# Contingencyy/CPUGPUPathtracing

Hardware: AMD Instinct MI355X
Metric: Mrays/sec @ 1920x1080, 256 spp (dragon glTF stand-in) (higher is better)
Workload: dtype f32

## Files before the change

cpugpupathtracing_amd/_native.py:

```python
from __future__ import annotations

import ctypes as C
import os

from ._paths import LIB_PATH

ABI_VERSION = 2
CGPT_OK, CGPT_ERR_INVALID, CGPT_ERR_HIP, CGPT_ERR_NO_SCENE, CGPT_ERR_UNSUPPORTED, CGPT_ERR_NO_DEVICE = range(6)
OBJECT_MESH, OBJECT_SPHERE, OBJECT_PLANE, OBJECT_TRIANGLE = 0, 1, 2, 3
MODE_COMPARISON, MODE_BRUTE_FORCE, MODE_ADVANCED = 0, 1, 2
DEBUG_NONE, DEBUG_RAY_DEPTH, DEBUG_BVH_DEPTH = 0, 1, 2
KERNEL_AUTO, KERNEL_MEGAKERNEL, KERNEL_WAVEFRONT, KERNEL_PERSISTENT = 0, 1, 2, 3
RENDER_COUNTERS = 1
CTX_FORCE_COLLECTIVE, CTX_GATHER_PEER_COPY = 1, 2
BUILD_NAIVE, BUILD_SAH_INTERVALS, BUILD_SAH_PRIMITIVES = 0, 1, 2
BUILD_SAH_BINNED = 3
DENOISE_DEMODULATE_ALBEDO = 1
TRACE_COUNTERS, TRACE_REVERSED = 1, 2
TEMPORAL_KEEP_VIEW_DEPENDENT = 1

f3 = C.c_float * 3


class Vertex(C.Structure):
# ... 145 lines not shown
    "cgpt_denoise": (C.c_int, [_vp, C.POINTER(Camera), C.POINTER(DenoiseParams), _fp, C.c_size_t, _up, C.c_size_t]),
    "cgpt_denoise_temporal": (C.c_int, [_vp, C.POINTER(Camera), C.POINTER(DenoiseParams), C.POINTER(TemporalParams), _fp, C.c_size_t, _up,
                                        C.c_size_t]),
    "cgpt_temporal_reset": (C.c_int, [_vp]),
    "cgpt_read_temporal_history": (C.c_int, [_vp, _fp, C.c_size_t]),
    "cgpt_measure_issue_rate": (C.c_int, [_vp, C.c_uint32, C.c_uint32, C.c_uint32, C.POINTER(C.c_double), C.POINTER(C.c_double)]),
    "cgpth_last_error": (C.c_char_p, []),
    "cgpth_mesh_load_gltf": (_vp, [C.c_char_p]),
    "cgpth_mesh_from_arrays": (_vp, [C.POINTER(Vertex), C.c_uint32, _up, C.c_uint32]),
    "cgpth_mesh_dragon_standin": (_vp, [C.c_uint32]),
    "cgpth_mesh_bumpy_icosphere": (_vp, [C.c_uint32, _fp, _fp, C.c_float]),
    "cgpth_mesh_save_gltf": (C.c_int, [_vp, C.c_char_p]),
    "cgpth_mesh_num_vertices": (C.c_uint32, [_vp]),
    "cgpth_mesh_num_indices": (C.c_uint32, [_vp]),
    "cgpth_mesh_vertices": (C.POINTER(Vertex), [_vp]),
    "cgpth_mesh_indices": (_up, [_vp]),
    "cgpth_mesh_free": (None, [_vp]),
    "cgpth_scene_new": (_vp, []),
    "cgpth_scene_free": (None, [_vp]),
    "cgpth_scene_reference_layout": (_vp, [_vp, C.c_uint32, C.c_float, C.c_int]),
    "cgpth_scene_add_material": (C.c_int, [_vp, C.POINTER(Material)]),
    "cgpth_scene_set_material": (C.c_int, [_vp, C.c_uint32, C.POINTER(Material)]),
    "cgpth_scene_set_roughness": (C.c_int, [_vp, C.c_uint32, C.c_float]),
    "cgpth_scene_get_roughness": (C.c_int, [_vp, _fp, C.c_uint32]),
    "cgpth_scene_set_transmission_roughness": (C.c_int, [_vp, C.c_uint32, C.c_float]),
    "cgpth_scene_get_transmission_roughness": (C.c_int, [_vp, _fp, C.c_uint32]),
    "cgpth_scene_add_mesh": (C.c_int, [_vp, _vp, C.c_uint32, C.c_int]),
    "cgpth_scene_add_mesh_device_built": (C.c_int, [_vp, _vp, C.c_uint32, _vp]),
    "cgpth_scene_add_mesh_device_built_ex": (C.c_int, [_vp, _vp, C.c_uint32, _vp, C.c_int]),
    "cgpth_scene_rebuild_bvh_device": (C.c_int, [_vp, C.c_uint32, C.c_int, _vp]),
    "cgpth_scene_add_sphere": (C.c_int, [_vp, _fp, C.c_float, C.c_uint32]),
    "cgpth_scene_add_plane": (C.c_int, [_vp, _fp, _fp, C.c_uint32]),
    "cgpth_scene_add_triangle": (C.c_int, [_vp, C.POINTER(Triangle), C.c_uint32]),
    "cgpth_scene_add_light": (C.c_int, [_vp, C.c_uint32]),
    "cgpth_scene_set_smooth_normals": (C.c_int, [_vp, C.c_uint32, C.c_uint32]),
    "cgpth_scene_get_smooth_normals": (C.c_int, [_vp, _up, C.c_uint32]),
    "cgpth_scene_set_transform": (C.c_int, [_vp, C.c_uint32, C.POINTER(C.c_float)]),
    "cgpth_scene_get_transforms": (C.c_int, [_vp, C.POINTER(C.c_float), C.c_uint32]),
    "cgpth_scene_set_camera": (C.c_int, [_vp, _fp, _fp, C.c_float, C.c_float]),
    "cgpth_scene_set_settings": (C.c_int, [_vp, C.POINTER(Settings)]),
    "cgpth_scene_rebuild_bvh": (C.c_int, [_vp, C.c_uint32, C.c_int]),
    "cgpth_scene_refit_mesh": (C.c_int, [_vp, C.c_uint32, C.POINTER(Triangle), C.c_uint32]),
    "cgpth_scene_update_primitive": (C.c_int, [_vp, C.c_uint32, C.POINTER(Object)]),
    "cgpth_scene_bvh_info": (C.c_int, [_vp, C.c_uint32, C.POINTER(BvhInfo)]),
    "cgpth_scene_bvh_export": (C.c_int, [_vp, C.c_uint32, C.POINTER(BvhNode), _up]),
    "cgpth_scene_flatten": (C.c_int, [_vp, C.POINTER(SceneDesc)]),
    "cgpth_scene_get_camera": (C.c_int, [_vp, C.POINTER(Camera)]),
    "cgpth_scene_get_settings": (C.c_int, [_vp, C.POINTER(Settings)]),
    "cgpth_write_ppm": (C.c_int, [C.c_char_p, _up, C.c_uint32, C.c_uint32]),
    "cgpth_write_pfm": (C.c_int, [C.c_char_p, _fp, C.c_uint32, C.c_uint32, C.c_uint32]),
    "cgpth_write_accumulator": (C.c_int, [C.c_char_p, _fp, C.c_uint32, C.c_uint32, C.c_uint32]),
    "cgpth_read_accumulator": (C.c_int, [C.c_char_p, _fp, _up, C.c_uint32, C.c_uint32]),
    "cgpth_fast_div": (C.c_uint32, [C.c_uint32, C.c_uint32]),
    "cgpth_scene_layout": (C.c_int, [C.POINTER(SceneDesc), C.POINTER(SceneLayoutView)]),
    "cgpth_scene_layout_transformed": (C.c_int, [C.POINTER(SceneDesc), C.POINTER(C.c_float), C.c_uint32, C.POINTER(SceneLayoutView)]),
    "cgpth_scene_permute_objects": (C.c_int, [_vp, _up, C.c_uint32]),
    "cgpth_top_level": (C.c_int, [C.POINTER(SceneDesc), C.POINTER(TopLevelView)]),
    "cgpth_top_level_transforms": (C.c_int, [C.POINTER(C.c_float), C.c_uint32, C.POINTER(TopLevelView)]),
    "cgpth_top_level_refit": (C.c_int, [C.c_uint32, C.POINTER(Triangle), C.c_uint32, C.POINTER(TopLevelView)]),
    "cgpth_top_level_primitive": (C.c_int, [C.c_uint32, C.POINTER(Object), C.POINTER(TopLevelView)]),
}

DEBUG_PROTOTYPES = {
    "cgpt_debug_live_device_bytes": (C.c_uint64, []),
}

_lib = None


class NativeLibraryError(RuntimeError):
    pass


def lib() -> C.CDLL:
    global _lib
    if _lib is not None:
        return _lib
    if not os.path.exists(LIB_PATH):
        raise NativeLibraryError(
            f"{LIB_PATH} is missing: run `python -m cpugpupathtracing_amd.build` (hipcc, gfx950). "
            "There is no CPU or Python fallback for the render path.")
    L = C.CDLL(LIB_PATH)
    for name, (restype, argtypes) in {**PROTOTYPES, **DEBUG_PROTOTYPES}.items():
        try:
            fn = getattr(L, name)
        except AttributeError as e:
            raise NativeLibraryError(f"{LIB_PATH} does not export {name}; rebuild it") from e
        fn.restype = restype
        fn.argtypes = argtypes
    if L.cgpt_abi_version() != ABI_VERSION:
        raise NativeLibraryError(f"ABI version mismatch: library reports {L.cgpt_abi_version()}, binding expects {ABI_VERSION}")
    _lib = L
    return L
```

cpugpupathtracing_amd/csrc/device/accumulate.hpp:

```cpp
#pragma once
#include <hip/hip_runtime.h>

#include "device_scene.h"
#include "rt_device.hpp"
#include "shade_device.hpp"
#include "trace_steps.hpp"

namespace cgpt {
namespace dev {

static constexpr uint32_t kAccChunk = 8;

__device__ __forceinline__ void accumulate_batch(const DevRenderArgs& args, const float4* __restrict__ st_en, const PathGrid& g,
                                                 uint32_t batch_first, uint32_t batch_n)
{
    __shared__ float4 stage[4][64 * (kAccChunk + 1u)];
    const DevSettings& st = args.settings;
    const uint32_t lane = threadIdx.x & 63u;
    float4* const my_stage = stage[threadIdx.x >> 6];
    double energy_sum = 0.0;
    for (uint32_t p = blockIdx.x * 256u + threadIdx.x; p < g.n_pixels; p += gridDim.x * 256u) {
        uint32_t px = 0, py = 0, local_row = 0;
        const bool is_pixel = pixel_of_index(args, g, p, px, py, local_row);
        const size_t local_index = (size_t)local_row * args.width + px;
        const bool brute = st.render_mode == 1u || (st.render_mode == 0u && px < args.width / 2u);
        float4 acc = is_pixel ? args.accumulator[local_index] : float4{ 0.0f, 0.0f, 0.0f, 0.0f };
        V3 last = mk(0.0f);
        auto add_sample = [&](float4 e4) {
            PathState ps;
            ps.energy = mk(e4.x, e4.y, e4.z);
            ps.depth = __float_as_uint(e4.w) & 0xFFu;
            const V3 e = brute ? ps.energy : final_energy(st, ps);
            energy_sum += (double)(e.x + e.y + e.z) * 0.001;
            if (st.debug_mode == 0u) { acc.x += e.x; acc.y += e.y; acc.z += e.z; acc.w += 1.0f; }
            else last = e;
        };
        if (g.order == kPixelMajor) {
            const uint32_t p_base = p - lane;
            for (uint32_t s0 = 0; s0 < batch_n; s0 += kAccChunk) {
                const uint32_t cnt = min(kAccChunk, batch_n - s0);
#pragma unroll
                for (uint32_t k = 0; k < kAccChunk; ++k) {
                    const uint32_t e = k * 64u + lane, pix = e / kAccChunk, smp = e % kAccChunk;
                    if (smp < cnt) my_stage[pix * (kAccChunk + 1u) + smp] = st_en[(size_t)(p_base + pix) * g.n_samples + s0 + smp];
                }
                __builtin_amdgcn_wave_barrier();
                if (is_pixel)
                    for (uint32_t j = 0; j < cnt; ++j) add_sample(my_stage[lane * (kAccChunk + 1u) + j]);
                __builtin_amdgcn_wave_barrier();
            }
        } else if (is_pixel) {
            for (uint32_t s = 0; s < batch_n; ++s) add_sample(ld_stream(&st_en[path_id(g, s, p)]));
        }
        if (is_pixel) {
            if (st.debug_mode == 0u) {
                args.accumulator[local_index] = acc;
                const float n = (float)(batch_first + batch_n);
                args.pixels[local_index] = vec4_to_uint(acc.x / n, acc.y / n, acc.z / n);
            } else {
                args.pixels[local_index] = vec4_to_uint(last.x, last.y, last.z);
            }
        }
    }
    block_add_f64(&args.counters->total_energy, energy_sum);
}

}
}
```

cpugpupathtracing_amd/csrc/device/wavefront_kernels.hip:

```cpp
#include <hip/hip_runtime.h>

#include <algorithm>
#include <cstdint>
#include <cstddef>
#include <cstdlib>
#include <cstring>
#include <new>
#include <type_traits>
#include <vector>

#include "cpugpupt_abi.h"
#include "ctx_internal.h"
#include "device_scene.h"
#include "fast_div.h"
#include "rt_device.hpp"
#include "shade_device.hpp"
#include "trace_steps.hpp"
#include "accumulate.hpp"
#include "launch_common.h"

namespace cgpt {

using namespace dev;

hipStream_t CtxStream(cgpt_ctx* ctx);
void** CtxWavefrontSlot(cgpt_ctx* ctx);
hipEvent_t CtxStartEvent(cgpt_ctx* ctx);

extern __shared__ uint32_t lds_dyn[];

static constexpr uint32_t kMaxBands = 128;

struct WfDev {
    float4* A; float4* B; float4* C;
    float4* st_tp; float4* st_en;
    float4* px_hit;
    float4* brute;
    uint8_t* hit_flag;
    uint32_t* list_ext; uint32_t* list_sh;
    uint32_t* seg_ext; uint32_t* seg_sh;
    uint32_t* seg_count;
    uint32_t* seg_prefix;
    uint32_t n_bands;
    uint32_t band_magic;
    uint32_t* plan;
    uint32_t* stack_overflow;
    uint32_t cap;
    uint32_t n_paths;
    PathGrid g;
    uint32_t n_segs, seg_cap;
    uint32_t shade_chunk;
    uint32_t retire_misses;
    uint32_t rot_trace[2], rot_shade;
    unsigned long long* spec_tab;
    uint32_t spec_keys;
    uint32_t spec_epoch;
    uint32_t probe;
};

static constexpr uint32_t kChainShift = 10u, kChainMax = 0xFFFFu, kFollowerBit = 0x80000000u, kNoLeader = 0xFFFFFFFFu;
static constexpr uint32_t kSameRayBit = 0x40000000u;

__device__ __forceinline__ uint32_t elect_chain_leader(const WfDev& wf, uint32_t chain, uint32_t pid)
{
    const bool want = chain != 0u;
    uint32_t pixel = 0;
    if (want) { uint32_t sample_unused; path_split(wf.g, pid, sample_unused, pixel); }
    uint32_t src = lane_id();
    for (unsigned long long pend = __builtin_amdgcn_ballot_w64(want); pend != 0ull;) {
// ... 155 lines not shown
                do {
                    if (r.code < kStartObject) inner_step<COUNT, STEP>(ctx, r, cnt);
                } while ((uint32_t)__popcll(__builtin_amdgcn_ballot_w64(r.code < kStartObject)) >= tune.inner_repeat);
            } else if (n_leaf >= w_obj) {
                do {
                    if ((int32_t)r.code < 0) leaf_step<COUNT, !FIRST, STEP>(ctx, r, cnt);
                } while ((uint32_t)__popcll(__builtin_amdgcn_ballot_w64((int32_t)r.code < 0)) >= tune.leaf_repeat);
            } else {
                do {
                    if (r.code == kStartObject && object_step<COUNT, !FIRST, XFORM, TREE>(ctx, r, cnt)) finish_ray();
                } while ((uint32_t)__popcll(__builtin_amdgcn_ballot_w64(r.code == kStartObject)) >= tune.obj_repeat);
            }
        }
    }

    const uint32_t per_ray = first_round ? wf.g.n_samples : 1u;
    if (first_round) wave_add_u64(&counters->traced_rays, cnt.rays, per_ray);
    else if (lane_id() == 0u && wave_rays) atomicAdd(&counters->traced_rays, (unsigned long long)wave_rays);
    if (!COUNT && !first_round && lane_id() == 0u && wave_followers) atomicAdd(&counters->chain_followers, (unsigned long long)wave_followers);
    if (!COUNT && !first_round && lane_id() == 0u && wave_unwalked) atomicAdd(&counters->retrace_unwalked, (unsigned long long)wave_unwalked);
    if (COUNT) {
        wave_add_u64(&counters->inner_steps, cnt.inner, per_ray);
        wave_add_u64(&counters->tri_tests, cnt.tris, per_ray);
        wave_add_u64(&counters->bvh_depth_sum, cnt.depth, per_ray);
    }
}

struct ShadeKernArgs { DevRenderArgs args; WfDev wf; uint32_t batch_first; };
static_assert(alignof(DevRenderArgs) == 8 && alignof(WfDev) == 8 && sizeof(DevRenderArgs) % 8 == 0, "ShadeKernArgs mirrors the argument segment: every parameter at its natural alignment");
__device__ __forceinline__ const ShadeKernArgs& shade_kernargs()
{
    const CGPT_UNIFORM ShadeKernArgs* p = (const CGPT_UNIFORM ShadeKernArgs*)__builtin_amdgcn_kernarg_segment_ptr();
    asm volatile("" : "+s"(p));
    return *(const ShadeKernArgs*)p;
}

template <bool COUNT, bool FIRST, bool BRUTE = false, int LOBES = 0, bool RIS = false>
__global__ void __launch_bounds__(256, 1) wf_shade(const DevRenderArgs, const WfDev, uint32_t)
{
    constexpr bool first_round = FIRST;
    constexpr bool kChains = !COUNT && !BRUTE;
    uint32_t n_ext;
    { const WfDev& wf = shade_kernargs().wf; n_ext = first_round ? wf.n_paths : wf.plan[0]; }
    const uint32_t n_blocks = (n_ext + 63u) / 64u;
    const uint32_t n_waves = gridDim.x * 4u;
    const uint32_t wave = blockIdx.x * 4u + __builtin_amdgcn_readfirstlane(threadIdx.x >> 6);
    uint32_t count_ext = 0, count_sh = 0;
    uint32_t cur_band = 0, band_start_ext = 0, band_start_sh = 0;
    Counters cnt = { 0, 0, 0, 0, 0, 0 };
    uint32_t wave_probed = 0;
    uint32_t wave_absorbed = 0;

    BlockWalk walk = first_block(wave);
    uint32_t block = wave * shade_kernargs().wf.shade_chunk;
    auto more = [&]() { return block < n_blocks; };
    auto advance = [&]() {
        const WfDev& wf = shade_kernargs().wf;
        const uint32_t chunk = wf.shade_chunk;
        if (++block >= min((block_of(walk) + 1u) * chunk, n_blocks)) {
            next_block(walk, n_waves, wf.rot_shade);
            block = block_of(walk) * chunk;
        }
    };
    __shared__ uint32_t s_queue[4][128];
    uint32_t* const queue = s_queue[threadIdx.x >> 6];
    uint32_t queued = 0;
    const bool hits_only = !first_round && shade_kernargs().wf.retire_misses != 0u;

    for (;;) {
        bool active = false;
        bool emit_ext = false, emit_sh = false;
        bool decided_sh = false, decided_ext = false;
        uint32_t pid = 0;
        uint32_t absorbed = 0;
        if (!hits_only) {
            if (!more()) break;
            const uint32_t i = block * 64u + lane_id();
            active = i < n_ext;
            if (active) pid = first_round ? i : ld_stream(&shade_kernargs().wf.list_ext[i]);
            advance();
        } else {
            while (queued < 64u && more()) {
                const WfDev& wf = shade_kernargs().wf;
                const uint32_t i = block * 64u + lane_id();
                uint32_t p = 0; bool hit = false;
                if (i < n_ext) { p = ld_stream(&wf.list_ext[i]); hit = wf.hit_flag[p] != 0; }
                const unsigned long long m = __builtin_amdgcn_ballot_w64(hit);
                if (hit) queue[queued + rank_in_mask(m)] = p;
                queued += (uint32_t)__popcll(m);
                advance();
            }
            if (queued == 0u) break;
            __builtin_amdgcn_wave_barrier();
            const uint32_t take = min(queued, 64u), rest = queued - take;
            active = lane_id() < take;
            if (active) pid = queue[lane_id()];
            const uint32_t moved = queue[64u + lane_id()];
            __builtin_amdgcn_wave_barrier();
            if (lane_id() < rest) queue[lane_id()] = moved;
            __builtin_amdgcn_wave_barrier();
            queued = rest;
        }
        float4 c;
        bool brute_path = false;
        uint32_t sample = 0, px = 0, py = 0;
        if (first_round && active) {
            const ShadeKernArgs& ka = shade_kernargs();
            const DevRenderArgs& args = ka.args;
            uint32_t pixel, local_row;
            path_split(ka.wf.g, pid, sample, pixel);
            active = pixel_of_index(args, ka.wf.g, pixel, px, py, local_row);
            if (active) {
                c = ka.wf.px_hit[pixel];
                if (BRUTE) brute_path = args.settings.render_mode == 1u || (args.settings.render_mode == 0u && px < args.width / 2u);
                if (__float_as_uint(c.x) == kNoHit && args.settings.debug_mode != 2u && !(BRUTE && brute_path)) {
                    float4 en; en.x = 0.0f; en.y = 0.0f; en.z = 0.0f; en.w = __uint_as_float(0u);
                    st_stream(&ka.wf.st_en[pid], en);
                    active = false;
                }
            }
        }
        if (active) {
            Ray ray, shadow;
            PathState ps;
            constexpr bool is_pixel = true;
            uint32_t chain = 0;
            bool followed = false;
            if (first_round) {
                const ShadeKernArgs& ka = shade_kernargs();
                const DevRenderArgs& args = ka.args;
                ps.rng = pcg_seed(py * args.width + px, ka.batch_first + sample, args.seed);
                ray = camera_ray(args.camera, (float)px * (1.0f / (float)args.width), (float)py * (1.0f / (float)args.height));
                ps.throughput = mk(1.0f); ps.energy = mk(0.0f); ps.depth = 0; ps.is_specular = false;
                chain = 1u;
            } else {
                const WfDev& wf = shade_kernargs().wf;
                const float4 a = ld_stream(&wf.A[pid]), b = ld_stream(&wf.B[pid]);
                ray.o = mk(a.x, a.y, a.z); ray.d = mk(b.x, b.y, b.z);
                const float4 tp = ld_stream(&wf.st_tp[pid]);
                ps.throughput = mk(tp.x, tp.y, tp.z); ps.rng = __float_as_uint(tp.w);
                ps.energy = mk(0.0f);
                const uint32_t fl = __float_as_uint(b.w);
                ps.depth = fl & 0xFFu; ps.is_specular = (fl & 0x100u) != 0u;
                if (BRUTE) brute_path = (fl & 0x200u) != 0u;
                if (kChains) chain = (fl >> kChainShift) & kChainMax;
                if (kChains && (fl & kFollowerBit)) {
                    const uint32_t lead = __float_as_uint(a.w);
                    followed = true;
                    if (!wf.retire_misses || wf.hit_flag[lead]) c = ld_stream(&wf.C[lead]);
                    else { c.x = __uint_as_float(kNoHit); c.y = 0.0f; c.z = 0.0f; c.w = 0.0f; }
                } else c = ld_stream(&wf.C[pid]);
            }
            ray.t = c.w; ray.obj = __float_as_uint(c.x); ray.tri = __float_as_uint(c.y); ray.bvh_depth = __float_as_uint(c.z);
            shadow = ray;
            V3 pending = mk(0.0f);

            uint32_t flags = kBounceTerminate;
            if (BRUTE && brute_path) {
                if (is_pixel) {
                    const ShadeKernArgs& ka = shade_kernargs();
                    const DevScene& sc = ka.args.scene;
                    const DevRenderArgs& args = ka.args;
                    const WfDev& wf = ka.wf;
                    const bool done = brute_level<COUNT, LOBES>(sc, args.settings, ray, ps.rng, ps.depth,
                        [&](uint32_t k, const BruteLevel& lv) {
                            float4* rec = wf.brute + ((size_t)k * wf.cap + pid) * 2u;
                            float4 r0, r1;
                            brute_pack(lv, r0, r1);
                            st_stream(&rec[0], r0); st_stream(&rec[1], r1);
                        },
// ... 155 lines not shown
    typedef uint32_t u4a4 __attribute__((ext_vector_type(4), aligned(4)));
    if (wf.n_bands == 1u) {
        for (uint32_t s = blockIdx.x; s < 2u * wf.n_segs; s += gridDim.x) {
            const bool sh = s >= wf.n_segs;
            const uint32_t seg = sh ? s - wf.n_segs : s;
            const uint32_t n = wf.seg_count[s], base = wf.seg_prefix[s];
            const uint32_t* src = (sh ? wf.seg_sh : wf.seg_ext) + (size_t)seg * wf.seg_cap;
            uint32_t* dst = (sh ? wf.list_sh : wf.list_ext) + base;
            const uint32_t n4 = n & ~3u;
            for (uint32_t i = threadIdx.x * 4u; i < n4; i += blockDim.x * 4u) *reinterpret_cast<u4a4*>(dst + i) = *reinterpret_cast<const u4a4*>(src + i);
            if (threadIdx.x < n - n4) dst[n4 + threadIdx.x] = src[n4 + threadIdx.x];
        }
        return;
    }
    __shared__ uint32_t s_n[kMaxBands], s_dst[kMaxBands], s_src[kMaxBands];
    const uint32_t lane = threadIdx.x & 63u, wave_in_block = threadIdx.x >> 6;
    for (uint32_t s = blockIdx.x; s < 2u * wf.n_segs; s += gridDim.x) {
        const bool sh = s >= wf.n_segs;
        const uint32_t seg = sh ? s - wf.n_segs : s;
        const uint32_t* cnt = wf.seg_count + (sh ? wf.n_bands * wf.n_segs : 0u);
        const uint32_t* pre = wf.seg_prefix + (sh ? wf.n_bands * wf.n_segs : 0u);
        const uint32_t* band_total = wf.plan + 2u + (sh ? wf.n_bands : 0u);
        __syncthreads();
        if (threadIdx.x < wf.n_bands) {
            s_n[threadIdx.x] = cnt[threadIdx.x * wf.n_segs + seg];
            s_dst[threadIdx.x] = pre[threadIdx.x * wf.n_segs + seg];
            s_src[threadIdx.x] = band_total[threadIdx.x];
        }
        __syncthreads();
        if (threadIdx.x == 0u) {
            uint32_t off = 0, base = 0;
            for (uint32_t b = 0; b < wf.n_bands; ++b) {
                const uint32_t n = s_n[b], total = s_src[b];
                s_dst[b] += base; s_src[b] = off;
                off += n; base += total;
            }
            if (seg == 0u) wf.plan[sh ? 1 : 0] = base;
        }
        __syncthreads();
        const uint32_t* src = (sh ? wf.seg_sh : wf.seg_ext) + (size_t)seg * wf.seg_cap;
        uint32_t* const list = sh ? wf.list_sh : wf.list_ext;
        for (uint32_t b = wave_in_block; b < wf.n_bands; b += 4u) {
            const uint32_t n = s_n[b], n4 = n & ~3u;
            uint32_t* dst = list + s_dst[b];
            const uint32_t* run = src + s_src[b];
            for (uint32_t i = lane * 4u; i < n4; i += 256u) *reinterpret_cast<u4a4*>(dst + i) = *reinterpret_cast<const u4a4*>(run + i);
            if (lane < n - n4) dst[n4 + lane] = run[n4 + lane];
        }
    }
}

__global__ void __launch_bounds__(256) wf_accumulate(const DevRenderArgs args, const WfDev wf, uint32_t batch_first, uint32_t batch_n)
{
    accumulate_batch(args, wf.st_en, wf.g, batch_first, batch_n);
}

static constexpr uint32_t kMaxPools = 8;

struct WfTuning {
    uint32_t pools = 8;
    uint32_t batch = 0;
    uint32_t max_batch = 512;
    uint32_t pool_paths_mi = 512;
    uint32_t budget_gib = 96;
    uint32_t refill_idle = 16;
    uint32_t leaf_repeat = 4;
    uint32_t inner_repeat = 20;
    uint32_t obj_repeat = 1;
    uint32_t obj_shift = 0;
    uint32_t top_records = kLdsTopMax;
    uint32_t max_trace_blocks = 64;
    uint32_t max_shade_blocks = 5;
    uint32_t shade_chunk = 4;
    uint32_t shade_chunk_banded = 32;
    uint32_t shadow_any_hit = 1;
    uint32_t lds_tris = 1;
    uint32_t first_lean = 1;
    uint32_t trace_events = 1;
    uint32_t path_order = 2;
    uint32_t retire_misses = 1;
    uint32_t bands_min_paths = 32u << 20;
    uint32_t bands = 32;
    uint32_t spec_dedupe = 1;
    uint32_t spec_keys = 8;
    uint32_t spec_epochs = 0xFFFF;
    uint32_t probe = 1;
    uint32_t probe_max_objects = 128;
};

static uint32_t Gcd(uint32_t a, uint32_t b) { while (b) { const uint32_t t = a % b; a = b; b = t; } return a; }
static uint32_t CoprimeRotation(uint32_t n_waves, uint32_t n_tiles)
{
    for (uint32_t rot = 0; rot < n_waves && rot < 4096u; ++rot)
        if (Gcd(n_waves + rot, std::max(1u, n_tiles)) == 1u) return rot;
    return 0u;
}

static decltype(&wf_trace<false, false>) const kTraceKernels[2][2][2] = {
    { { wf_trace<false, false>, wf_trace<false, true> }, { wf_trace<true, false>, wf_trace<true, true> } },
    { { wf_trace<false, false, true>, wf_trace<false, true, true> }, { wf_trace<true, false, true>, wf_trace<true, true, true> } },
};
static decltype(&wf_trace<false, false>) const kTraceTreeKernels[2][2][2] = {
    { { wf_trace<false, false, false, true>, wf_trace<false, true, false, true> }, { wf_trace<true, false, false, true>, wf_trace<true, true, false, true> } },
    { { wf_trace<false, false, true, true>, wf_trace<false, true, true, true> }, { wf_trace<true, false, true, true>, wf_trace<true, true, true, true> } },
};
#define CGPT_SHADE_LEVEL(G, R) \
    { { { wf_shade<false, false, false, G, R>, wf_shade<false, false, true, G, R> }, { wf_shade<false, true, false, G, R>, wf_shade<false, true, true, G, R> } }, \
// ... 209 lines not shown
    const uint32_t n_pixels = (uint32_t)n_pixels64;
    const uint32_t rounds = (uint32_t)args_in.settings.max_ray_depth + 2u;

    const bool xform = HonoursTransforms((int)v.lobe_level);
    h->last_xform = xform;
    const bool tree = v.tree;
    h->last_tree = tree;
    TraceLaunch tl;
    if (PrepareTraceLaunch(ctx, h, args_in.scene, xform, count, tree, tl) != 0) return -1;
    const uint32_t n_cus = h->n_cus;
    const dim3 block(256);
    const auto& trace_kernels = tl.kernels;
    const size_t trace_lds = tl.lds;
    const dim3 trace_grid_first = tl.grid_first, trace_grid_later = tl.grid_later;
    const bool brute = args_in.settings.render_mode != 2u;
    const uint32_t brute_levels = brute ? (uint32_t)args_in.settings.max_ray_depth + 1u : 0u;
    uint32_t shade_blocks[2][2];
    for (int c = 0; c < 2; ++c)
        for (int b = 0; b < 2; ++b) shade_blocks[c][b] = std::min(h->tune.max_shade_blocks, h->shade_blocks_per_cu[v.ris][v.lobe_level][c][b]);
    const dim3 shade_grid(n_cus * shade_blocks[count][brute]);
    const uint32_t n_segs = n_cus * std::max({ shade_blocks[0][0], shade_blocks[1][0], shade_blocks[0][1], shade_blocks[1][1] }) * 4u;
    const uint32_t min_shade_waves = n_cus * std::min({ shade_blocks[0][0], shade_blocks[1][0], shade_blocks[0][1], shade_blocks[1][1] }) * 4u;

    const uint32_t overflow_words = tl.overflow_words;

    uint32_t shade_chunk = h->tune.shade_chunk;
    const bool chains = h->tune.spec_dedupe && !count && !brute;
    const size_t spec_entries = chains ? (size_t)n_pixels * h->tune.spec_keys : 0u;
    const size_t kBytesPerPath = 160 + 32 * (size_t)brute_levels;
    size_t free_b = 0, total_b = 0;
    LAUNCH_TRY(hipMemGetInfo(&free_b, &total_b));
    const size_t held_bytes = (size_t)h->held_pools * PoolBytes(h->held);
    const size_t budget = std::min<size_t>((size_t)h->tune.budget_gib << 30, (free_b + held_bytes) / 2);
    uint32_t batch = h->tune.batch;
    if (batch == 0) {
        batch = 1;
        while (batch < h->tune.max_batch && (uint64_t)n_pixels * batch * 2u <= (uint64_t)pool_paths) batch *= 2u;
    }
    batch = std::max(1u, std::min({ batch, std::max(1u, args_in.n_samples / 2u), args_in.n_samples, pool_paths / n_pixels }));
    WfSizes need;
    need.n_pixels = n_pixels; need.n_segs = n_segs; need.overflow_words = overflow_words; need.brute_levels = brute_levels; need.spec = spec_entries;
    uint32_t n_pools = 0, n_batches = 0;
    for (int attempt = 0;; ++attempt) {
        for (;;) {
            need.cap = n_pixels * batch;
            n_batches = (args_in.n_samples + batch - 1u) / batch;
            const uint32_t afford = (uint32_t)std::min<size_t>(kMaxPools, budget / ((size_t)need.cap * kBytesPerPath + spec_entries * sizeof(unsigned long long)));
            n_pools = std::max(1u, std::min({ h->tune.pools, n_batches, afford }));
            if (batch == 1u || (afford >= 1u && n_pools >= std::min({ 2u, n_batches, h->tune.pools }))) break;
            batch /= 2u;
        }
        const bool banded = h->tune.bands > 1u && need.cap >= h->tune.bands_min_paths;
        shade_chunk = banded ? h->tune.shade_chunk_banded : h->tune.shade_chunk;
        need.seg_cap = ((((need.cap + 63u) / 64u + shade_chunk - 1u) / shade_chunk + min_shade_waves - 1u) / min_shade_waves) * shade_chunk * 64u;
        if (h->held_pools >= n_pools && h->held.Holds(need)) break;
        LAUNCH_TRY(hipDeviceSynchronize());
        WfRelease(h);
        hipError_t err = hipSuccess;
        for (uint32_t p = 0; p < n_pools; ++p) {
            WfDev& d = h->dev[p];
            ForEachBuffer(d, need, [&](auto*& ptr, size_t bytes) { if (err == hipSuccess && bytes) err = DevAlloc((void**)&ptr, bytes); });
            if (err == hipSuccess && d.spec_tab) err = hipMemset(d.spec_tab, 0, need.spec * sizeof(unsigned long long));
            h->spec_epoch[p] = 0;
        }
        if (err == hipSuccess) { h->held = need; h->held_pools = n_pools; break; }
        (void)hipGetLastError();
        WfRelease(h);
        if (batch == 1u || attempt >= 8) { CtxFail(ctx, CGPT_ERR_HIP, "wavefront pools: %s", hipGetErrorString(err)); return -1; }
        batch /= 2u;
    }

    if (ReserveEvents(ctx, h->trace_ev, 2u * n_batches * rounds) != 0) return -1;
    h->trace_rounds = rounds;

    LAUNCH_TRY(hipEventRecord(CtxStartEvent(ctx), stream));
    LAUNCH_TRY(hipEventRecord(h->begin, stream));
    for (uint32_t p = 0; p < n_pools; ++p) LAUNCH_TRY(hipStreamWaitEvent(h->streams[p], h->begin, 0));

    int launches = 0;
    DevRenderArgs args = args_in;
    const TraceTune tt = tl.tune;
    uint32_t k = 0;
    for (uint32_t done = 0; done < args_in.n_samples; done += batch, ++k) {
        const uint32_t p = k % n_pools;
        hipStream_t st = h->streams[p];
        const uint32_t bn = std::min(batch, args_in.n_samples - done);
        const uint32_t bfirst = args_in.first_sample + done;
        WfDev wf = h->dev[p];
        wf.cap = h->held.cap; wf.n_paths = n_pixels * bn;
        wf.rot_trace[0] = CoprimeRotation(trace_grid_later.x * (kTraceBlock / 64u), tiles_x * tiles_y);
        wf.rot_trace[1] = CoprimeRotation(trace_grid_first.x * (kTraceBlock / 64u), tiles_x * tiles_y);
        wf.rot_shade = CoprimeRotation(shade_grid.x * 4u, std::max(1u, tiles_x * tiles_y / shade_chunk));
        wf.shade_chunk = shade_chunk;
        wf.g = MakePathGrid(n_pixels, tiles_x, bn, h->tune.path_order); wf.n_segs = h->held.n_segs; wf.seg_cap = h->held.seg_cap;
        wf.n_bands = h->tune.bands > 1u && wf.n_paths >= h->tune.bands_min_paths ? h->tune.bands : 1u;
        if (wf.n_bands > 1u)
            wf.band_magic = (uint32_t)std::min<uint64_t>(0xFFFFFFFFull, (((uint64_t)wf.n_bands << 32) + wf.n_paths - 1u) / wf.n_paths);
        wf.retire_misses = h->tune.retire_misses && args_in.settings.debug_mode == 0u ? 1u : 0u;
        if (!chains) wf.spec_tab = nullptr;
        wf.spec_keys = h->tune.spec_keys;
        wf.probe = h->tune.probe && !count && !xform && !tree && args_in.settings.debug_mode == 0u && args_in.scene.n_objects <= h->tune.probe_max_objects ? 1u : 0u;
        if (k < n_pools) LAUNCH_TRY(hipMemsetAsync(wf.seg_count, 0, 2 * (size_t)kMaxBands * wf.n_segs * sizeof(uint32_t), st));
        for (uint32_t r = 0; r < rounds; ++r) {
            const bool first = r == 0u;
            if (h->tune.trace_events) LAUNCH_TRY(hipEventRecord(NextEvent(h->trace_ev), st));
            hipLaunchKernelGGL(trace_kernels[xform][count][first], first ? trace_grid_first : trace_grid_later, dim3(kTraceBlock), trace_lds, st, args, wf, bfirst, tt);
            if (h->tune.trace_events) LAUNCH_TRY(hipEventRecord(NextEvent(h->trace_ev), st));
// ... 207 lines not shown
```

cpugpupathtracing_amd/csrc/host/host_capi.cpp:

```cpp
#include <cstring>
#include <exception>
#include <new>
#include <string>

#include "cpugpupt_host.h"
#include "fast_div.h"
#include "gltf_loader.h"
#include "image_io.h"
#include "mesh_gen.h"
#include "scene.h"
#include "transform_math.h"

using namespace cgpt;

struct cgpth_mesh { Mesh mesh; };
struct cgpth_scene {
    Scene scene;
    Scene::FlatStorage flat;
};

namespace {
thread_local std::string g_error;
int Fail(const std::string& msg) { g_error = msg; return CGPT_ERR_INVALID; }
Vec3 V(const float p[3]) { return { p[0], p[1], p[2] }; }

Material FromAbi(const cgpt_material& m)
{
    Material out;
    out.albedo = V(m.albedo); out.specular = m.specular; out.refractivity = m.refractivity;
    out.absorption = V(m.absorption); out.ior = m.ior; out.emissive = V(m.emissive);
    out.intensity = m.intensity; out.is_light = m.is_light != 0;
    return out;
}
bool ValidOption(int o) { return o >= 0 && o < MeshBVH::BuildOption_NumOptions; }

template <class R, class F>
R Guarded(R on_error, F&& body) noexcept
{
    try {
        return body();
    } catch (const std::exception& e) {
        try { g_error = std::string("exception in the host mirror: ") + e.what(); } catch (...) {}
    } catch (...) {
        try { g_error = "unknown exception in the host mirror"; } catch (...) {}
    }
    return on_error;
}
}

namespace cgpt {
void HostSetError(const char* msg) { try { g_error = msg; } catch (...) {} }
}

extern "C" {

const char* cgpth_last_error(void) { return g_error.c_str(); }

cgpth_mesh* cgpth_mesh_load_gltf(const char* path)
{
    return Guarded<cgpth_mesh*>(nullptr, [&]() -> cgpth_mesh* {
        if (!path) { Fail("null path"); return nullptr; }
        cgpth_mesh* m = new (std::nothrow) cgpth_mesh;
        if (!m) { Fail("out of memory"); return nullptr; }
// ... 423 lines not shown
int cgpth_scene_get_camera(const cgpth_scene* scene, cgpt_camera* out)
{
    return Guarded<int>((int)CGPT_ERR_INVALID, [&]() -> int {
        if (!scene || !out) return Fail("null argument");
        *out = scene->scene.camera.Abi();
        return CGPT_OK;
    });
}

int cgpth_scene_get_settings(const cgpth_scene* scene, cgpt_settings* out)
{
    return Guarded<int>((int)CGPT_ERR_INVALID, [&]() -> int {
        if (!scene || !out) return Fail("null argument");
        *out = scene->scene.AbiSettings();
        return CGPT_OK;
    });
}

int cgpth_write_ppm(const char* path, const uint32_t* pixels, uint32_t width, uint32_t height)
{
    return Guarded<int>((int)CGPT_ERR_INVALID, [&]() -> int {
        std::string err;
        if (!path || !pixels) return Fail("null argument");
        return WritePPM(path, pixels, width, height, err) ? CGPT_OK : Fail(err);
    });
}
int cgpth_write_pfm(const char* path, const float* acc, uint32_t n, uint32_t width, uint32_t height)
{
    return Guarded<int>((int)CGPT_ERR_INVALID, [&]() -> int {
        std::string err;
        if (!path || !acc) return Fail("null argument");
        return WritePFM(path, acc, n, width, height, err) ? CGPT_OK : Fail(err);
    });
}
int cgpth_write_accumulator(const char* path, const float* acc, uint32_t n, uint32_t width, uint32_t height)
{
    return Guarded<int>((int)CGPT_ERR_INVALID, [&]() -> int {
        std::string err;
        if (!path || !acc) return Fail("null argument");
        return WriteAccumulator(path, acc, n, width, height, err) ? CGPT_OK : Fail(err);
    });
}
int cgpth_read_accumulator(const char* path, float* acc, uint32_t* n, uint32_t width, uint32_t height)
{
    return Guarded<int>((int)CGPT_ERR_INVALID, [&]() -> int {
        std::string err;
        if (!path || !acc || !n) return Fail("null argument");
        return ReadAccumulator(path, acc, n, width, height, err) ? CGPT_OK : Fail(err);
    });
}

uint32_t cgpth_fast_div(uint32_t n, uint32_t d) { return d == 0u ? 0u : fast_div(n, MakeFastDiv(d)); }

}
```

include/cpugpupt_host.h:

```cpp
#ifndef CPUGPUPT_HOST_H
#define CPUGPUPT_HOST_H

#include "cpugpupt_abi.h"

#ifdef __cplusplus
extern "C" {
#endif

enum cgpth_build_option { CGPTH_BUILD_NAIVE = 0, CGPTH_BUILD_SAH_INTERVALS = 1, CGPTH_BUILD_SAH_PRIMITIVES = 2,
                          CGPTH_BUILD_SAH_BINNED = 3  };

typedef struct cgpth_mesh cgpth_mesh;
typedef struct cgpth_scene cgpth_scene;

typedef struct cgpth_bvh_info {
    uint32_t num_triangles, nodes_used, num_leaves, max_leaf_size, max_depth;
    float total_area;
} cgpth_bvh_info;

const char* cgpth_last_error(void);

cgpth_mesh* cgpth_mesh_load_gltf(const char* path);
cgpth_mesh* cgpth_mesh_from_arrays(const cgpt_vertex* vertices, uint32_t n_vertices, const uint32_t* indices, uint32_t n_indices);
cgpth_mesh* cgpth_mesh_dragon_standin(uint32_t level);
cgpth_mesh* cgpth_mesh_bumpy_icosphere(uint32_t level, const float center[3], const float radii[3], float bump);
int cgpth_mesh_save_gltf(const cgpth_mesh* mesh, const char* gltf_path);
uint32_t cgpth_mesh_num_vertices(const cgpth_mesh* mesh);
uint32_t cgpth_mesh_num_indices(const cgpth_mesh* mesh);
const cgpt_vertex* cgpth_mesh_vertices(const cgpth_mesh* mesh);
const uint32_t* cgpth_mesh_indices(const cgpth_mesh* mesh);
void cgpth_mesh_free(cgpth_mesh* mesh);

cgpth_scene* cgpth_scene_new(void);
void cgpth_scene_free(cgpth_scene* scene);
cgpth_scene* cgpth_scene_reference_layout(const cgpth_mesh* mesh, uint32_t mesh_material, float aspect, int build_option);
int cgpth_scene_add_material(cgpth_scene* scene, const cgpt_material* material);
int cgpth_scene_set_material(cgpth_scene* scene, uint32_t index, const cgpt_material* material);
int cgpth_scene_set_roughness(cgpth_scene* scene, uint32_t index, float roughness);
int cgpth_scene_get_roughness(const cgpth_scene* scene, float* out, uint32_t n);
int cgpth_scene_set_transmission_roughness(cgpth_scene* scene, uint32_t index, float transmission_roughness);
int cgpth_scene_get_transmission_roughness(const cgpth_scene* scene, float* out, uint32_t n);
int cgpth_scene_add_mesh(cgpth_scene* scene, const cgpth_mesh* mesh, uint32_t mat_index, int build_option);
int cgpth_scene_add_mesh_device_built(cgpth_scene* scene, const cgpth_mesh* mesh, uint32_t mat_index, cgpt_ctx* ctx);
int cgpth_scene_add_mesh_device_built_ex(cgpth_scene* scene, const cgpth_mesh* mesh, uint32_t mat_index, cgpt_ctx* ctx, int build_option);
int cgpth_scene_add_sphere(cgpth_scene* scene, const float center[3], float radius, uint32_t mat_index);
int cgpth_scene_add_plane(cgpth_scene* scene, const float normal[3], const float point[3], uint32_t mat_index);
int cgpth_scene_add_triangle(cgpth_scene* scene, const cgpt_triangle* triangle, uint32_t mat_index);
int cgpth_scene_add_light(cgpth_scene* scene, uint32_t obj_index);
int cgpth_scene_set_smooth_normals(cgpth_scene* scene, uint32_t obj_index, uint32_t flag);
int cgpth_scene_get_smooth_normals(const cgpth_scene* scene, uint32_t* out, uint32_t n);
int cgpth_scene_set_transform(cgpth_scene* scene, uint32_t obj_index, const float object_to_world[12]);
int cgpth_scene_get_transforms(const cgpth_scene* scene, float* out, uint32_t n);
int cgpth_scene_set_camera(cgpth_scene* scene, const float pos[3], const float view_dir[3], float fov_deg, float aspect);
int cgpth_scene_set_settings(cgpth_scene* scene, const cgpt_settings* settings);
int cgpth_scene_rebuild_bvh(cgpth_scene* scene, uint32_t obj_index, int build_option);
int cgpth_scene_rebuild_bvh_device(cgpth_scene* scene, uint32_t obj_index, int build_option, cgpt_ctx* ctx);
int cgpth_scene_refit_mesh(cgpth_scene* scene, uint32_t obj_index, const cgpt_triangle* triangles, uint32_t n_tris);
int cgpth_scene_update_primitive(cgpth_scene* scene, uint32_t obj_index, const cgpt_object* obj);
int cgpth_scene_permute_objects(cgpth_scene* scene, const uint32_t* order, uint32_t n_objects);
int cgpth_scene_bvh_info(const cgpth_scene* scene, uint32_t obj_index, cgpth_bvh_info* out);
int cgpth_scene_bvh_export(const cgpth_scene* scene, uint32_t obj_index, cgpt_bvh_node* nodes, uint32_t* tri_indices);
int cgpth_scene_flatten(cgpth_scene* scene, cgpt_scene_desc* out);
int cgpth_scene_get_camera(const cgpth_scene* scene, cgpt_camera* out);
int cgpth_scene_get_settings(const cgpth_scene* scene, cgpt_settings* out);

int cgpth_write_ppm(const char* path, const uint32_t* pixels, uint32_t width, uint32_t height);
int cgpth_write_pfm(const char* path, const float* accumulator_rgba, uint32_t num_accumulated, uint32_t width, uint32_t height);
int cgpth_write_accumulator(const char* path, const float* accumulator_rgba, uint32_t num_accumulated, uint32_t width, uint32_t height);
int cgpth_read_accumulator(const char* path, float* accumulator_rgba, uint32_t* num_accumulated, uint32_t width, uint32_t height);

uint32_t cgpth_fast_div(uint32_t n, uint32_t d);

typedef struct cgpth_scene_layout_view {
    const float* node_pairs; size_t n_node_pairs;
    const float* tri_leaf; size_t n_tri_leaf;
    const float* tri_orig; size_t n_tri_orig;
    const float* tri_normal; size_t n_tri_normal;
    const float* materials; size_t n_materials;
    const float* obj_trace; size_t n_obj_trace;
    const void* objects; size_t n_objects; size_t object_size;
    const uint32_t* lights; size_t n_lights;
    const uint32_t* refit_levels; size_t n_refit_levels;
    const uint32_t* record_perm; size_t n_record_perm;
    uint32_t stack_depth, n_top_records, n_pair_records, n_small_tris;
    const uint32_t* leaf_base; const uint32_t* pair_base; const uint32_t* level_begin;
    const uint32_t* level_offsets; const uint32_t* level_offsets_start;
    const float* tri_normal12; size_t n_tri_normal12;
    const float* obj_xform; size_t n_obj_xform;
} cgpth_scene_layout_view;
int cgpth_scene_layout(const cgpt_scene_desc* scene, cgpth_scene_layout_view* out);
int cgpth_scene_layout_transformed(const cgpt_scene_desc* scene, const float* object_to_world, uint32_t n_objects, cgpth_scene_layout_view* out);

typedef struct cgpth_top_level_view {
    const float* nodes; size_t n_nodes;
    const uint32_t* entry; size_t n_entry;
} cgpth_top_level_view;
int cgpth_top_level(const cgpt_scene_desc* scene, cgpth_top_level_view* out);
int cgpth_top_level_transforms(const float* object_to_world, uint32_t n_objects, cgpth_top_level_view* out);
int cgpth_top_level_refit(uint32_t obj_index, const cgpt_triangle* triangles, uint32_t n_tris, cgpth_top_level_view* out);
int cgpth_top_level_primitive(uint32_t obj_index, const cgpt_object* obj, cgpth_top_level_view* out);

#ifdef __cplusplus
}
#endif
#endif
```

Baseline: 21750.

## Adapt shade work-item size and skip energy traffic for empty non-brute pixels

The shade kernel now picks a per-wave work-item size (in blocks) from the live block count, shrinking the chunk when there are too few blocks to give every wave a full chunk, so load balances better at low occupancy. Separately, for advanced-mode pixels whose primary ray missed, the shade kernel no longer writes zero energy records and the accumulate kernel skips reading them, substituting a zero record instead. This removes memory traffic for background pixels, at the cost of an extra px_hit read and a ballot in accumulate.

```diff
diff --git a/cpugpupathtracing_amd/_native.py b/cpugpupathtracing_amd/_native.py
--- a/cpugpupathtracing_amd/_native.py
+++ b/cpugpupathtracing_amd/_native.py
@@ -221,6 +221,8 @@
     "cgpth_write_accumulator": (C.c_int, [C.c_char_p, _fp, C.c_uint32, C.c_uint32, C.c_uint32]),
     "cgpth_read_accumulator": (C.c_int, [C.c_char_p, _fp, _up, C.c_uint32, C.c_uint32]),
     "cgpth_fast_div": (C.c_uint32, [C.c_uint32, C.c_uint32]),
+    "cgpth_shade_item_blocks": (C.c_uint32, [C.c_uint32, C.c_uint32, C.c_uint32]),
+    "cgpth_shade_segment_blocks": (C.c_uint32, [C.c_uint32, C.c_uint32, C.c_uint32]),
     "cgpth_scene_layout": (C.c_int, [C.POINTER(SceneDesc), C.POINTER(SceneLayoutView)]),
     "cgpth_scene_layout_transformed": (C.c_int, [C.POINTER(SceneDesc), C.POINTER(C.c_float), C.c_uint32, C.POINTER(SceneLayoutView)]),
     "cgpth_scene_permute_objects": (C.c_int, [_vp, _up, C.c_uint32]),
diff --git a/cpugpupathtracing_amd/csrc/device/accumulate.hpp b/cpugpupathtracing_amd/csrc/device/accumulate.hpp
--- a/cpugpupathtracing_amd/csrc/device/accumulate.hpp
+++ b/cpugpupathtracing_amd/csrc/device/accumulate.hpp
@@ -11,8 +11,16 @@
 
 static constexpr uint32_t kAccChunk = 8;
 
+__device__ __forceinline__ bool pixel_adds_nothing(const DevRenderArgs& args, float4 first_hit, uint32_t px)
+{
+    const DevSettings& st = args.settings;
+    const bool trace_path = st.render_mode == 1u || (st.render_mode == 0u && px < args.width / 2u);
+    return __float_as_uint(first_hit.x) == kNoHit && st.debug_mode == 0u && !trace_path;
+}
+
+template <bool SKIP = false>
 __device__ __forceinline__ void accumulate_batch(const DevRenderArgs& args, const float4* __restrict__ st_en, const PathGrid& g,
-                                                 uint32_t batch_first, uint32_t batch_n)
+                                                 uint32_t batch_first, uint32_t batch_n, const float4* __restrict__ px_hit = nullptr)
 {
     __shared__ float4 stage[4][64 * (kAccChunk + 1u)];
     const DevSettings& st = args.settings;
@@ -35,22 +43,26 @@
             if (st.debug_mode == 0u) { acc.x += e.x; acc.y += e.y; acc.z += e.z; acc.w += 1.0f; }
             else last = e;
         };
+        bool nothing = false;
+        if (SKIP && is_pixel) nothing = pixel_adds_nothing(args, px_hit[p], px);
+        const float4 zero_record = float4{ 0.0f, 0.0f, 0.0f, __uint_as_float(0u) };
         if (g.order == kPixelMajor) {
             const uint32_t p_base = p - lane;
+            const unsigned long long unread = SKIP ? __builtin_amdgcn_ballot_w64(nothing) : 0ull;
             for (uint32_t s0 = 0; s0 < batch_n; s0 += kAccChunk) {
                 const uint32_t cnt = min(kAccChunk, batch_n - s0);
 #pragma unroll
                 for (uint32_t k = 0; k < kAccChunk; ++k) {
                     const uint32_t e = k * 64u + lane, pix = e / kAccChunk, smp = e % kAccChunk;
-                    if (smp < cnt) my_stage[pix * (kAccChunk + 1u) + smp] = st_en[(size_t)(p_base + pix) * g.n_samples + s0 + smp];
+                    if (smp < cnt && !(SKIP && ((unread >> pix) & 1ull))) my_stage[pix * (kAccChunk + 1u) + smp] = st_en[(size_t)(p_base + pix) * g.n_samples + s0 + smp];
                 }
                 __builtin_amdgcn_wave_barrier();
                 if (is_pixel)
-                    for (uint32_t j = 0; j < cnt; ++j) add_sample(my_stage[lane * (kAccChunk + 1u) + j]);
+                    for (uint32_t j = 0; j < cnt; ++j) add_sample(SKIP && nothing ? zero_record : my_stage[lane * (kAccChunk + 1u) + j]);
                 __builtin_amdgcn_wave_barrier();
             }
         } else if (is_pixel) {
-            for (uint32_t s = 0; s < batch_n; ++s) add_sample(ld_stream(&st_en[path_id(g, s, p)]));
+            for (uint32_t s = 0; s < batch_n; ++s) add_sample(SKIP && nothing ? zero_record : ld_stream(&st_en[path_id(g, s, p)]));
         }
         if (is_pixel) {
             if (st.debug_mode == 0u) {
diff --git a/cpugpupathtracing_amd/csrc/device/shade_items.h b/cpugpupathtracing_amd/csrc/device/shade_items.h
--- /dev/null
+++ b/cpugpupathtracing_amd/csrc/device/shade_items.h
@@ -0,0 +1,30 @@
+#pragma once
+#include <cstdint>
+
+#include "fast_div.h"
+
+namespace cgpt {
+
+CGPT_HD inline uint32_t shade_wave_blocks(uint32_t n_blocks, uint32_t n_waves, uint32_t item)
+{
+    const uint32_t items = (n_blocks + item - 1u) / item;
+    return ((items + n_waves - 1u) / n_waves) * item;
+}
+
+CGPT_HD inline uint32_t shade_segment_blocks(uint32_t cap_blocks, uint32_t min_waves, uint32_t chunk)
+{
+    return shade_wave_blocks(cap_blocks, min_waves, chunk);
+}
+
+static constexpr uint32_t kShadeItemMin = 4;
+
+CGPT_HD inline uint32_t shade_item_blocks(uint32_t n_blocks, uint32_t n_waves, uint32_t chunk)
+{
+    if ((uint64_t)n_blocks >= (uint64_t)n_waves * chunk) return chunk;
+    uint32_t k = 0;
+    while ((2u << k) <= chunk && (((uint64_t)n_waves << (k + 1u)) <= n_blocks || (2u << k) <= kShadeItemMin)) ++k;
+    while (k > 0u && (uint64_t)((n_blocks + (1u << k) - 1u) >> k) > (uint64_t)(chunk >> k) * n_waves) --k;
+    return (1u << k) >= kShadeItemMin ? 1u << k : chunk;
+}
+
+}
diff --git a/cpugpupathtracing_amd/csrc/device/wavefront_kernels.hip b/cpugpupathtracing_amd/csrc/device/wavefront_kernels.hip
--- a/cpugpupathtracing_amd/csrc/device/wavefront_kernels.hip
+++ b/cpugpupathtracing_amd/csrc/device/wavefront_kernels.hip
@@ -15,6 +15,7 @@
 #include "fast_div.h"
 #include "rt_device.hpp"
 #include "shade_device.hpp"
+#include "shade_items.h"
 #include "trace_steps.hpp"
 #include "accumulate.hpp"
 #include "launch_common.h"
@@ -276,13 +277,12 @@
     uint32_t wave_absorbed = 0;
 
     BlockWalk walk = first_block(wave);
-    uint32_t block = wave * shade_kernargs().wf.shade_chunk;
+    const uint32_t chunk = shade_item_blocks(n_blocks, n_waves, shade_kernargs().wf.shade_chunk);
+    uint32_t block = wave * chunk;
     auto more = [&]() { return block < n_blocks; };
     auto advance = [&]() {
-        const WfDev& wf = shade_kernargs().wf;
-        const uint32_t chunk = wf.shade_chunk;
         if (++block >= min((block_of(walk) + 1u) * chunk, n_blocks)) {
-            next_block(walk, n_waves, wf.rot_shade);
+            next_block(walk, n_waves, shade_kernargs().wf.rot_shade);
             block = block_of(walk) * chunk;
         }
     };
@@ -338,8 +338,10 @@
                 c = ka.wf.px_hit[pixel];
                 if (BRUTE) brute_path = args.settings.render_mode == 1u || (args.settings.render_mode == 0u && px < args.width / 2u);
                 if (__float_as_uint(c.x) == kNoHit && args.settings.debug_mode != 2u && !(BRUTE && brute_path)) {
-                    float4 en; en.x = 0.0f; en.y = 0.0f; en.z = 0.0f; en.w = __uint_as_float(0u);
-                    st_stream(&ka.wf.st_en[pid], en);
+                    if (!pixel_adds_nothing(args, c, px)) {
+                        float4 en; en.x = 0.0f; en.y = 0.0f; en.z = 0.0f; en.w = __uint_as_float(0u);
+                        st_stream(&ka.wf.st_en[pid], en);
+                    }
                     active = false;
                 }
             }
@@ -601,7 +603,7 @@
 
 __global__ void __launch_bounds__(256) wf_accumulate(const DevRenderArgs args, const WfDev wf, uint32_t batch_first, uint32_t batch_n)
 {
-    accumulate_batch(args, wf.st_en, wf.g, batch_first, batch_n);
+    accumulate_batch<true>(args, wf.st_en, wf.g, batch_first, batch_n, wf.px_hit);
 }
 
 static constexpr uint32_t kMaxPools = 8;
@@ -917,7 +919,7 @@
         }
         const bool banded = h->tune.bands > 1u && need.cap >= h->tune.bands_min_paths;
         shade_chunk = banded ? h->tune.shade_chunk_banded : h->tune.shade_chunk;
-        need.seg_cap = ((((need.cap + 63u) / 64u + shade_chunk - 1u) / shade_chunk + min_shade_waves - 1u) / min_shade_waves) * shade_chunk * 64u;
+        need.seg_cap = shade_segment_blocks((need.cap + 63u) / 64u, min_shade_waves, shade_chunk) * 64u;
         if (h->held_pools >= n_pools && h->held.Holds(need)) break;
         LAUNCH_TRY(hipDeviceSynchronize());
         WfRelease(h);
diff --git a/cpugpupathtracing_amd/csrc/host/host_capi.cpp b/cpugpupathtracing_amd/csrc/host/host_capi.cpp
--- a/cpugpupathtracing_amd/csrc/host/host_capi.cpp
+++ b/cpugpupathtracing_amd/csrc/host/host_capi.cpp
@@ -9,6 +9,7 @@
 #include "image_io.h"
 #include "mesh_gen.h"
 #include "scene.h"
+#include "shade_items.h"
 #include "transform_math.h"
 
 using namespace cgpt;
@@ -538,4 +539,7 @@
 
 uint32_t cgpth_fast_div(uint32_t n, uint32_t d) { return d == 0u ? 0u : fast_div(n, MakeFastDiv(d)); }
 
-}
+uint32_t cgpth_shade_item_blocks(uint32_t n_blocks, uint32_t n_waves, uint32_t chunk) { return n_waves == 0u || chunk == 0u ? 0u : shade_item_blocks(n_blocks, n_waves, chunk); }
+uint32_t cgpth_shade_segment_blocks(uint32_t cap_blocks, uint32_t min_waves, uint32_t chunk) { return min_waves == 0u || chunk == 0u ? 0u : shade_segment_blocks(cap_blocks, min_waves, chunk); }
+
+}
diff --git a/include/cpugpupt_host.h b/include/cpugpupt_host.h
--- a/include/cpugpupt_host.h
+++ b/include/cpugpupt_host.h
@@ -71,6 +71,9 @@
 
 uint32_t cgpth_fast_div(uint32_t n, uint32_t d);
 
+uint32_t cgpth_shade_item_blocks(uint32_t n_blocks, uint32_t n_waves, uint32_t chunk);
+uint32_t cgpth_shade_segment_blocks(uint32_t cap_blocks, uint32_t min_waves, uint32_t chunk);
+
 typedef struct cgpth_scene_layout_view {
     const float* node_pairs; size_t n_node_pairs;
     const float* tri_leaf; size_t n_tri_leaf;
```

Measured after the change: 22330, median of 6. 1.03x the previous value.
